# WoodOxen/tactics2d

Measured on NVIDIA H100. Metric: participant_steps_per_sec, higher is better.
Workload: dtype f32

## Files before the change

### tactics2d_b200/csrc/t2d_kernels.cu

```cuda
#include <cuda_runtime.h>
#include <stdint.h>
#include <stdio.h>
#include <string.h>

#include <algorithm>
#include <atomic>
#include <cmath>
#include <memory>
#include <mutex>
#include <string>
#include <vector>

#include "../../include/t2d_b200.h"
#include "t2d_math.cuh"

namespace t2d {

constexpr int MAX_WARPS_PER_CTA = 8;
constexpr int CTA_THREADS = MAX_WARPS_PER_CTA * 32;
constexpr int PPL = 4;
constexpr int POSE_PER_WARP = 32 * PPL;
constexpr int MAP_SMEM_LIMIT = 120 * 1024;

struct MapHeader {
// ... 13 lines not shown
  uint32_t smem_bytes;
  float bxmin, bxmax, bymin, bymax;
  int32_t has_bounds;
  uint32_t pad[3];
};
constexpr float CLEAR_QUANT = 0.125f;
static_assert(sizeof(MapHeader) == 128, "MapHeader must be 128 bytes");

struct WorldArgs {
  float *x, *y, *h, *v, *vx, *vy;
  const uint8_t* type_id;
  int32_t* step_count;
  const Params* table;
  int n_types, N, M;
};

struct MapArgs {
  const unsigned char* map_blob;
  const uint32_t* tile_off;
  const uint16_t* tile_id;
};

__device__ __forceinline__ const unsigned char* tile_blob(const MapArgs& m, long long n) {
  return m.map_blob ? m.map_blob + (m.tile_id ? m.tile_off[m.tile_id[n]] : 0u) : nullptr;
}

struct GoalArgs {
  const float* target;
  float* iou;
  float* last_pose;
  int32_t* noact_count;
  float threshold;
  int noact_max;
};

struct StepArgs {
  float *x, *y, *h, *v, *vx, *vy;
  const uint8_t* type_id;
  int32_t* step_count;
  const float* action;
  const float* ego_action;
  uint8_t* flags;
  int16_t* hit_index;
  int16_t* hit_segment;
  uint8_t* scn_status;
  uint8_t* done;
  const unsigned char* map_blob;
  const uint32_t* tile_off;
  const uint16_t* tile_id;
  MapHeader mh;
  const Params* table;
  int map_bytes, map_in_smem;
  int n_types;
  int N, M, G;
  int g_shift, mp_shift, unused1, n_tiles, wpc, table_bytes;
  int off_poseA, off_poseB, off_hit, off_queue, off_sorted, unused0, off_qcount, off_bar;
  int n_steps;
  float dt, dt_rem;
  double dt_d, dt_rem_d, interval_d;
  int max_step, cfg_flags;
  int do_physics, has_bounds, vec_ok, needs_vel_in;
  int prefetch;
  float bxmin, bxmax, bymin, bymax;
  float rb_max;
  GoalArgs goal;
  float *wheel_f, *wheel_r;
};

__device__ __forceinline__ uint32_t smem_u32(const void* p) { return (uint32_t)__cvta_generic_to_shared(p); }

__device__ __forceinline__ void mbar_init(uint64_t* bar, uint32_t count) {
  asm volatile("mbarrier.init.shared::cta.b64 [%0], %1;" ::"r"(smem_u32(bar)), "r"(count));
}
__device__ __forceinline__ void fence_mbar_init() { asm volatile("fence.mbarrier_init.release.cluster;" ::: "memory"); }
__device__ __forceinline__ void mbar_expect_tx(uint64_t* bar, uint32_t bytes) {
  asm volatile("mbarrier.arrive.expect_tx.shared::cta.b64 _, [%0], %1;" ::"r"(smem_u32(bar)), "r"(bytes) : "memory");
}
__device__ __forceinline__ void bulk_g2s(void* dst, const void* src, uint32_t bytes, uint64_t* bar) {
  asm volatile("cp.async.bulk.shared::cluster.global.mbarrier::complete_tx::bytes [%0], [%1], %2, [%3];" ::"r"(
                   smem_u32(dst)),
               "l"(src), "r"(bytes), "r"(smem_u32(bar))
               : "memory");
}
__device__ __forceinline__ void mbar_wait(uint64_t* bar, uint32_t parity) {
  uint32_t ok = 0;
  while (!ok) {
    asm volatile(
        "{\n\t.reg .pred p;\n\t"
        "mbarrier.try_wait.parity.shared::cta.b64 p, [%1], %2;\n\t"
        "selp.u32 %0, 1, 0, p;\n\t}"
        : "=r"(ok)
        : "r"(smem_u32(bar)), "r"(parity)
        : "memory");
  }
}

template <int BYTES> struct VecOf;
template <> struct VecOf<1> { using T = uint8_t; };
template <> struct VecOf<2> { using T = uint16_t; };
template <> struct VecOf<4> { using T = uint32_t; };
template <> struct VecOf<8> { using T = uint2; };
template <> struct VecOf<16> { using T = uint4; };

template <typename T, int N>
__device__ __forceinline__ void ld_vec(const T* p, T (&o)[N]) {
  using V = typename VecOf<sizeof(T) * N>::T;
  const V v = *reinterpret_cast<const V*>(p);
  memcpy(o, &v, sizeof(V));
}
template <typename T, int N>
__device__ __forceinline__ void st_vec(T* p, const T (&o)[N]) {
  using V = typename VecOf<sizeof(T) * N>::T;
  V v;
  memcpy(&v, o, sizeof(V));
  *reinterpret_cast<V*>(p) = v;
}

struct Pose {
  float x, y, h, c, s, l, w;
};

__device__ __noinline__ bool pair_exact(const Pose a, const Pose b) {
  const bool ca = a.w < 0.0f, cb = b.w < 0.0f;
  if (!ca && !cb) return obb_obb_f64(a.x, a.y, a.h, a.l, a.w, b.x, b.y, b.h, b.l, b.w);
  if (!ca && cb) return obb_circle_f64(a.x, a.y, a.h, a.l, a.w, b.x, b.y, b.l);
  if (ca && !cb) return obb_circle_f64(b.x, b.y, b.h, b.l, b.w, a.x, a.y, a.l);
  return circle_circle_f64(a.x, a.y, a.l, b.x, b.y, b.l);
}

__device__ __forceinline__ bool pair_hit(const Pose& a, const Pose& b) {
  const bool ca = a.w < 0.0f, cb = b.w < 0.0f;
  int r;
  if (!ca && !cb) r = obb_obb_f32(a.x, a.y, a.c, a.s, a.l, a.w, b.x, b.y, b.c, b.s, b.l, b.w);
  else if (!ca && cb) r = obb_circle_f32(a.x, a.y, a.c, a.s, a.l, a.w, b.x, b.y, b.l);
  else if (ca && !cb) r = obb_circle_f32(b.x, b.y, b.c, b.s, b.l, b.w, a.x, a.y, a.l);
  else r = circle_circle_f32(a.x, a.y, a.l, b.x, b.y, b.l);
  if (r < 0) return pair_exact(a, b);
  return r != 0;
}

__device__ __noinline__ bool seg_exact(const Pose a, const float4 sg) {
  if (a.w < 0.0f) return circle_segment_f64(a.x, a.y, a.l, sg.x, sg.y, sg.z, sg.w);
  return obb_segment_f64(a.x, a.y, a.h, a.l, a.w, sg.x, sg.y, sg.z, sg.w);
}

__device__ __forceinline__ bool seg_hit(const Pose& a, const float4 sg) {
  int r = a.w < 0.0f ? circle_segment_f32(a.x, a.y, a.l, sg.x, sg.y, sg.z, sg.w)
                     : obb_segment_f32(a.x, a.y, a.c, a.s, a.l, a.w, sg.x, sg.y, sg.z, sg.w);
  if (r < 0) return seg_exact(a, sg);
  return r != 0;
}

__device__ __noinline__ bool oob_exact(const Pose a, float xmin, float xmax, float ymin, float ymax) {
  return out_of_bound_f64(a.x, a.y, a.h, a.l, a.w, a.w < 0.0f, xmin, xmax, ymin, ymax);
}

__device__ __noinline__ void other_model_step(OneIO& io, const Params& p, int n_steps, double dt, double dt_rem, double interval) {
  if (p.model() == MODEL_DYNAMICS) {
    dynamics_step(io, p, n_steps, dt);
  } else if (p.model() == MODEL_POINTMASS_NEWTON) {
    pointmass_newton_step(io, p, interval);
  } else if (p.model() == MODEL_POINTMASS_EULER) {
    pointmass_euler_step(io, p, n_steps, dt, dt_rem);
  } else {
    sincos_fast(io.h, &io.sh, &io.ch);
  }
// ... 206 lines not shown
    return t;
  };
  __syncwarp();
  for (int k = lane; k < base; k += 32) {
    const int ti = (int)queue[k];
    const TileRef t = tile_of(ti);
    const Pose a = load_pose(poseA, poseB, ti);
    const int best = t.mh->n_seg > 0 ? static_walk(ti, a, poseA[pslot(ti)].z, *t.mh, map_view(t.sec, *t.mh), queue, qcount) : 0x7fffffff;
    segmin[pslot(ti)] = best;
  }
  __syncwarp();
  const int n_x = min(*qcount, QCAP - QX0);
  for (int k = lane; k < n_x; k += 32) {
    const unsigned e = queue[QX0 + k];
    const int ti = (int)(e >> 16), sidx = (int)(e & 0xffffu);
    int* sm = &segmin[pslot(ti)];
    if (*sm != -2 && sidx < *sm) {
      const TileRef t = tile_of(ti);
      if (seg_exact(load_pose(poseA, poseB, ti), reinterpret_cast<const float4*>(t.sec + t.mh->off_seg)[sidx])) atomicMin(sm, sidx);
    }
  }
  __syncwarp();
  for (int k = lane; k < base; k += 32) {
    const int ti = (int)queue[k];
    int* sm = &segmin[pslot(ti)];
    const TileRef t = tile_of(ti);
    if (*sm == -2) {
      const MapView mv = map_view(t.sec, *t.mh);
      *sm = static_walk_exact(load_pose(poseA, poseB, ti), poseA[pslot(ti)].z, *t.mh, mv.seg, mv.cell_start, mv.items);
    }
    if (t.mh->n_poly > 0) {
      const float4 pa = poseA[pslot(ti)];
      *sm = static_objects(*sm, pa.x, pa.y, *t.mh, t.blob);
    }
  }
  __syncwarp();
}

__device__ __noinline__ bool oob_slow(const float4* poseA, const float4* poseB, int idx, float xmin, float xmax, float ymin, float ymax) {
  const Pose a = load_pose(poseA, poseB, idx);
  int r = out_of_bound_f32(a.x, a.y, a.c, a.s, a.l, a.w, a.w < 0.0f, xmin, xmax, ymin, ymax);
  if (r < 0) r = out_of_bound_f64(a.x, a.y, a.h, a.l, a.w, a.w < 0.0f, xmin, xmax, ymin, ymax) ? 1 : 0;
  return r != 0;
}

template <class Args>
__device__ __noinline__ unsigned ego_goal_events(const Args& A, long long n, float ex, float ey, float eh, float el, float ew) {
  const GoalArgs& G = A.goal;
  unsigned r = 0;
  float* last = G.last_pose + 4 * n;
  if (G.noact_max > 0) {
    int cnt = G.noact_count[n];
    if (last[3] != 0.0f) {
      const double iou = rect_iou_f64(ex, ey, eh, el, ew, last[0], last[1], last[2], el, ew);
      cnt = iou > 0.999 ? cnt + 1 : 0;
    }
    G.noact_count[n] = cnt;
    if (cnt > G.noact_max) r |= 2u;
  }
  last[0] = ex; last[1] = ey; last[2] = eh; last[3] = 1.0f;
  const float* tg = G.target + 5 * n;
  const double iou = rect_iou_f64(ex, ey, eh, el, ew, tg[0], tg[1], tg[2], tg[3], tg[4]);
  G.iou[n] = (float)iou;
  if (iou >= (double)G.threshold) r |= 1u;
  return r;
}

constexpr int FIX_M = 64, FIX_G = 16, FIX_G_SHIFT = 4, FIX_MP_SHIFT = 6;

template <bool FIXED>
__device__ __forceinline__ void prefetch_tile_l2(const StepArgs& A, long long i) {
  asm volatile("prefetch.global.L2 [%0];" ::"l"(A.x + i));
  asm volatile("prefetch.global.L2 [%0];" ::"l"(A.y + i));
  asm volatile("prefetch.global.L2 [%0];" ::"l"(A.h + i));
  asm volatile("prefetch.global.L2 [%0];" ::"l"(A.v + i));
  if (FIXED || A.action) asm volatile("prefetch.global.L2 [%0];" ::"l"(A.action + 2 * i));
  asm volatile("prefetch.global.L2 [%0];" ::"l"(A.type_id + i));
  if (!FIXED && A.needs_vel_in) {
    asm volatile("prefetch.global.L2 [%0];" ::"l"(A.vx + i));
    asm volatile("prefetch.global.L2 [%0];" ::"l"(A.vy + i));
  }
}

#ifdef T2D_TICK_TIMELINE
constexpr int TL_POINTS = 9, TL_MAX_WARPS = 4096;
__device__ unsigned long long t2d_timeline[TL_MAX_WARPS][TL_POINTS][2];
#define T2D_TL(k, on, slot, dep)                                                                                    \
  do {                                                                                                              \
    if ((on) && (slot) < TL_MAX_WARPS) {                                                                            \
      unsigned long long g_, c_;                                                                                    \
      asm volatile("mov.u64 %0, %%globaltimer;\n\tmov.u64 %1, %%clock64;" : "=l"(g_), "=l"(c_) : "f"(dep) : "memory"); \
      t2d_timeline[slot][k][0] = g_;                                                                                \
      t2d_timeline[slot][k][1] = c_;                                                                                \
    }                                                                                                               \
  } while (0)
#else
#define T2D_TL(k, on, slot, dep)
#endif

template <bool KIN_ONLY, bool MAP_TABLE, bool FIXED>
__global__ void __launch_bounds__(CTA_THREADS, 2) t2d_step_kernel(const __grid_constant__ StepArgs A) {
  extern __shared__ __align__(128) unsigned char smem[];
  T2D_TL(0, (threadIdx.x & 31) == 0, (int)(blockIdx.x * A.wpc + (threadIdx.x >> 5)), 0.0f);
  const int map_smem_bytes = (!MAP_TABLE && A.map_in_smem) ? A.map_bytes : 0;
  const int table_bytes = A.table_bytes;
  const int wpc = A.wpc;
  unsigned char* s_map = smem;
  Params* s_table = reinterpret_cast<Params*>(smem + map_smem_bytes);
  float4* s_poseA = reinterpret_cast<float4*>(smem + A.off_poseA);
  float4* s_poseB = reinterpret_cast<float4*>(smem + A.off_poseB);
  int* s_hit = reinterpret_cast<int*>(smem + A.off_hit);
  unsigned* s_queue = reinterpret_cast<unsigned*>(smem + A.off_queue);
  float4* s_sorted = reinterpret_cast<float4*>(smem + A.off_sorted);
  int* s_qcount = reinterpret_cast<int*>(smem + A.off_qcount);
  uint64_t* s_bar = reinterpret_cast<uint64_t*>(smem + A.off_bar);

  const int tid = threadIdx.x, lane = tid & 31, warp = tid >> 5;
  asm volatile("griddepcontrol.launch_dependents;" ::: "memory");

  if (tid == 0) {
    mbar_init(s_bar, 1);
    fence_mbar_init();
  }
  __syncthreads();
  if (tid == 0) {
    mbar_expect_tx(s_bar, (uint32_t)(table_bytes + map_smem_bytes));
    bulk_g2s(s_table, A.table, (uint32_t)table_bytes, s_bar);
    if (map_smem_bytes > 0) bulk_g2s(s_map, A.map_blob, (uint32_t)map_smem_bytes, s_bar);
  }
  bool staged = false;
#define K1_SHAPE(field, fixed_value) (FIXED ? (fixed_value) : A.field)
  {
    const long long n_ = ((long long)blockIdx.x * wpc + warp) * (32 >> K1_SHAPE(g_shift, FIX_G_SHIFT)) + (lane >> K1_SHAPE(g_shift, FIX_G_SHIFT));
    const int m_ = (lane & (K1_SHAPE(G, FIX_G) - 1)) * PPL;
    if (A.prefetch && n_ < A.N && m_ < K1_SHAPE(M, FIX_M)) prefetch_tile_l2<FIXED>(A, n_ * K1_SHAPE(M, FIX_M) + m_);
  }
  asm volatile("griddepcontrol.wait;" ::: "memory");
  T2D_TL(1, lane == 0, (int)blockIdx.x * wpc + warp, 0.0f);
  const int G = K1_SHAPE(G, FIX_G), M = K1_SHAPE(M, FIX_M);
  const int spw = 32 >> K1_SHAPE(g_shift, FIX_G_SHIFT);
  const int sub = lane >> K1_SHAPE(g_shift, FIX_G_SHIFT);
  const int gl = lane & (G - 1);
  const int m0 = gl * PPL;
  const int MP = G * PPL;
  float4* poseA = s_poseA + warp * POSE_PER_WARP;
  float4* poseB = s_poseB + warp * POSE_PER_WARP;
  int* hitmin = s_hit + warp * POSE_PER_WARP;
  unsigned* queue = s_queue + warp * QCAP;
  int* qcount = s_qcount + warp;
  const int tb = sub * MP, t0 = tb + m0;
  const int mp_shift = K1_SHAPE(mp_shift, FIX_MP_SHIFT);
  float4* sorted = s_sorted + warp * POSE_PER_WARP + tb;
  const int Mh = M >> 1;

  const int n_tiles = A.n_tiles;
  for (int tile = (int)blockIdx.x * wpc + warp; tile < n_tiles; tile += (int)gridDim.x * wpc) {
    const long long n = (long long)tile * spw + sub;
    const bool scn_ok = n < A.N;
    int nvalid = scn_ok ? (FIXED ? PPL : min(PPL, M - m0)) : 0;
    if (nvalid < 0) nvalid = 0;
    const long long idx0 = n * M + m0;
#ifdef T2D_TICK_TIMELINE
    const bool tl_on = lane == 0 && tile == (int)blockIdx.x * wpc + warp;
    const int tl_slot = tile;
#endif

    float sx[PPL], sy[PPL], shd[PPL], sv[PPL], svx[PPL], svy[PPL], a0[PPL], a1[PPL];
    int tidv[PPL];
#pragma unroll
    for (int i = 0; i < PPL; ++i) {
      sx[i] = sy[i] = shd[i] = sv[i] = svx[i] = svy[i] = a0[i] = a1[i] = 0.0f;
      tidv[i] = T2D_TYPE_INACTIVE;
    }
    if (nvalid == PPL && K1_SHAPE(vec_ok, 1)) {
      ld_vec<float, PPL>(A.x + idx0, sx);
      ld_vec<float, PPL>(A.y + idx0, sy);
      ld_vec<float, PPL>(A.h + idx0, shd);
      ld_vec<float, PPL>(A.v + idx0, sv);
      uint8_t tb8[PPL];
      ld_vec<uint8_t, PPL>(A.type_id + idx0, tb8);
#pragma unroll
      for (int i = 0; i < PPL; ++i) tidv[i] = tb8[i];
      if (K1_SHAPE(do_physics, 1)) {
        float2 act[PPL];
        float lo[4], hi[4];
        ld_vec<float, 4>(A.action + 2 * idx0, lo);
        ld_vec<float, 4>(A.action + 2 * idx0 + 4, hi);
        act[0] = make_float2(lo[0], lo[1]); act[1] = make_float2(lo[2], lo[3]);
        act[2] = make_float2(hi[0], hi[1]); act[3] = make_float2(hi[2], hi[3]);
#pragma unroll
        for (int i = 0; i < PPL; ++i) { a0[i] = act[i].x; a1[i] = act[i].y; }
        if (K1_SHAPE(needs_vel_in, 0)) {
          ld_vec<float, PPL>(A.vx + idx0, svx);
          ld_vec<float, PPL>(A.vy + idx0, svy);
        }
      }
    } else {
#pragma unroll
      for (int i = 0; i < PPL; ++i) {
        if (i < nvalid) {
          sx[i] = A.x[idx0 + i]; sy[i] = A.y[idx0 + i]; shd[i] = A.h[idx0 + i]; sv[i] = A.v[idx0 + i];
          tidv[i] = A.type_id[idx0 + i];
          if (K1_SHAPE(do_physics, 1)) {
            a0[i] = A.action[2 * (idx0 + i)]; a1[i] = A.action[2 * (idx0 + i) + 1];
            if (K1_SHAPE(needs_vel_in, 0)) { svx[i] = A.vx[idx0 + i]; svy[i] = A.vy[idx0 + i]; }
          }
        }
      }
    }
    {
      const long long n_next = n + (long long)gridDim.x * wpc * spw;
      if (A.prefetch && n_next < A.N && m0 < M) prefetch_tile_l2<FIXED>(A, n_next * M + m0);
    }
    if (K1_SHAPE(ego_action, nullptr) != nullptr && K1_SHAPE(do_physics, 1) && gl == 0 && scn_ok) {
      const float2 ea = reinterpret_cast<const float2*>(K1_SHAPE(ego_action, nullptr))[n];
      a0[0] = ea.x; a1[0] = ea.y;
    }
    if (!staged) {
      mbar_wait(s_bar, 0);
      staged = true;
    }
    float ch[PPL], sh[PPL];
    bool active[PPL], kin[PPL];
    const Params* pp[PPL];
    int model[PPL];
    bool lane_all_kin = true, lane_any_kin = false;
#pragma unroll
    for (int i = 0; i < PPL; ++i) {
      active[i] = tidv[i] < A.n_types;
      pp[i] = &s_table[active[i] ? tidv[i] : 0];
      model[i] = pp[i]->model_shape & 0xff;
      kin[i] = active[i] && (model[i] == MODEL_KINEMATICS);
      lane_all_kin = lane_all_kin && kin[i];
      lane_any_kin = lane_any_kin || kin[i];
      ch[i] = 1.0f; sh[i] = 0.0f;
    }
    T2D_TL(2, tl_on, tl_slot, sx[PPL - 1] + sy[PPL - 1] + shd[PPL - 1] + sv[PPL - 1] + a0[PPL - 1] + a1[PPL - 1] + (float)model[PPL - 1]);
    if (A.cfg_flags & T2D_CFG_STEER_FIRST) {
#pragma unroll
      for (int i = 0; i < PPL; ++i)
        if (model[i] <= MODEL_DYNAMICS || model[i] == MODEL_DRIFT) { float t = a0[i]; a0[i] = a1[i]; a1[i] = t; }
    }

    if (K1_SHAPE(do_physics, 1)) {
      if (__any_sync(0xffffffffu, lane_any_kin)) {
        const Params* const null_row = &s_table[A.n_types];
        const Params* pk[PPL];
        KinIO<PPL> io;
#pragma unroll
        for (int i = 0; i < PPL; ++i) {
          pk[i] = kin[i] ? pp[i] : null_row;
          io.x[i] = kin[i] ? sx[i] : 0.0f; io.y[i] = kin[i] ? sy[i] : 0.0f;
          io.h[i] = kin[i] ? shd[i] : 0.0f; io.v[i] = kin[i] ? sv[i] : 0.0f;
          io.acc[i] = kin[i] ? a0[i] : 0.0f; io.steer[i] = kin[i] ? a1[i] : 0.0f;
        }
        kinematics_step<PPL>(io, pk, A.n_steps, A.dt, A.dt_rem);
#pragma unroll
// ... 186 lines not shown
        if (((solid_bits >> i) & 1u) && near_decide(near_q[i], near_alt[i], rb[i])) near_bits |= 1u << i;
      if (__any_sync(0xffffffffu, near_bits != 0)) {
        static_phase<MAP_TABLE>(near_bits, t0, lane, tile * spw, mp_shift, A, s_map, poseA, poseB, hitmin, queue, qcount);
#pragma unroll
        for (int i = 0; i < PPL; ++i) {
          const int h = hitmin[i * 32 + lane];
          hseg[i] = (h == 0x7fffffff) ? -1 : h;
        }
      }
    }
    T2D_TL(7, tl_on, tl_slot, (float)(hseg[0] + hseg[PPL - 1]));

    float bxmin = A.bxmin, bxmax = A.bxmax, bymin = A.bymin, bymax = A.bymax;
    bool has_bounds = A.has_bounds != 0;
    if constexpr (MAP_TABLE) {
      has_bounds = lane_mh->has_bounds != 0;
      bxmin = lane_mh->bxmin; bxmax = lane_mh->bxmax; bymin = lane_mh->bymin; bymax = lane_mh->bymax;
    }
    uint8_t fl[PPL];
    unsigned oob_check = 0;
#pragma unroll
    for (int i = 0; i < PPL; ++i) {
      uint8_t f = 0;
      if (hit[i] >= 0) f |= T2D_F_DYNAMIC;
      if (hseg[i] >= 0) f |= T2D_F_STATIC;
      const float r = rb[i] * 1.0001f + 1e-3f;
      const bool clear_in = (px[i] - bxmin > r) && (bxmax - px[i] > r) && (py[i] - bymin > r) && (bymax - py[i] > r);
      if (has_bounds && ((solid_bits >> i) & 1u) && !clear_in) oob_check |= 1u << i;
      fl[i] = f;
    }
    if (oob_check) {
#pragma unroll
      for (int i = 0; i < PPL; ++i)
        if (((oob_check >> i) & 1u) && oob_slow(poseA, poseB, t0 + i, bxmin, bxmax, bymin, bymax)) fl[i] |= T2D_F_OUTBOUND;
    }
    if (nvalid == PPL && K1_SHAPE(vec_ok, 1)) {
      int16_t h16[PPL], s16[PPL];
#pragma unroll
      for (int i = 0; i < PPL; ++i) { h16[i] = (int16_t)hit[i]; s16[i] = (int16_t)hseg[i]; }
      if (A.flags) st_vec<uint8_t, PPL>(A.flags + idx0, fl);
      if (A.hit_index) st_vec<int16_t, PPL>(A.hit_index + idx0, h16);
      if (A.hit_segment) st_vec<int16_t, PPL>(A.hit_segment + idx0, s16);
    } else {
#pragma unroll
      for (int i = 0; i < PPL; ++i) {
        if (i < nvalid) {
          if (A.flags) A.flags[idx0 + i] = fl[i];
          if (A.hit_index) A.hit_index[idx0 + i] = (int16_t)hit[i];
          if (A.hit_segment) A.hit_segment[idx0 + i] = (int16_t)hseg[i];
        }
      }
    }

    if (K1_SHAPE(do_physics, 1)) {
      unsigned agg;
      if (A.cfg_flags & T2D_CFG_ANY_PARTICIPANT) {
        agg = 0;
#pragma unroll
        for (int i = 0; i < PPL; ++i) agg |= fl[i];
        for (int o = G >> 1; o > 0; o >>= 1) agg |= __shfl_xor_sync(0xffffffffu, agg, o);
      } else {
        agg = __shfl_sync(0xffffffffu, (unsigned)fl[0], sub * G);
      }
      if (gl == 0 && scn_ok) {
        const int cnt = cnt_in + 1;
        A.step_count[n] = cnt;
        uint8_t st = T2D_STATUS_NORMAL;
        unsigned goal = 0;
        if (K1_SHAPE(goal.target, nullptr) != nullptr) {
          const float4 ea = poseA[pslot(t0)], eb = poseB[pslot(t0)];
          if (ea.x == ea.x && eb.w >= 0.0f) goal = ego_goal_events(A, n, ea.x, ea.y, ea.w, eb.z, eb.w);
        }
        if (goal & 1u) st = T2D_STATUS_COMPLETED;
        if (agg & T2D_F_DYNAMIC) st = T2D_STATUS_FAILED;
        if (agg & T2D_F_STATIC) st = T2D_STATUS_FAILED;
        if (agg & T2D_F_OUTBOUND) st = T2D_STATUS_OUT_BOUND;
        if (goal & 2u) st = T2D_STATUS_NO_ACTION;
        if (A.max_step > 0 && cnt > A.max_step) st = T2D_STATUS_TIME_EXCEEDED;
        if (A.scn_status) A.scn_status[n] = st;
        if (A.done) A.done[n] = st != T2D_STATUS_NORMAL;
      }
    }
    T2D_TL(8, tl_on, tl_slot, 0.0f);
    __syncwarp();
  }
  if (!staged) mbar_wait(s_bar, 0);
#undef K1_SHAPE
}

struct ResetArgs : WorldArgs {
  const uint8_t* mask;
  const int32_t* pool_index;
  const float *px, *py, *ph, *pv, *pvx, *pvy;
  GoalArgs goal;
  float *wheel_f, *wheel_r;
  const float *pool_wf, *pool_wr;
  float* last_accel;
  int n_pool;
  uint8_t* agent_type_id;
  uint8_t* agent_retired;
  GoalArgs agent;
  int agent_q;
};

__global__ void t2d_reset_kernel(const __grid_constant__ ResetArgs A) {
  const long long total = (long long)A.N * A.M;
  for (long long i = (long long)blockIdx.x * blockDim.x + threadIdx.x; i < total; i += (long long)gridDim.x * blockDim.x) {
    const int n = (int)(i / A.M), m = (int)(i - (long long)n * A.M);
    if (!A.mask[n]) continue;
    int r = A.pool_index ? A.pool_index[n] : n;
    r = min(max(r, 0), A.n_pool - 1);
    const long long s = (long long)r * A.M + m;
    A.x[i] = A.px[s]; A.y[i] = A.py[s]; A.h[i] = A.ph[s]; A.v[i] = A.pv[s];
    A.vx[i] = A.pvx ? A.pvx[s] : A.pv[s] * cosf(A.ph[s]);
    A.vy[i] = A.pvy ? A.pvy[s] : A.pv[s] * sinf(A.ph[s]);
    if (A.agent_type_id != nullptr) {
      const uint8_t rt = A.agent_retired[i];
      if (rt != 0xff) { A.agent_type_id[i] = rt; A.agent_retired[i] = 0xff; }
      for (int q = m; q < A.agent_q; q += A.M) {
        A.agent.last_pose[4 * ((long long)n * A.agent_q + q) + 3] = 0.0f;
        A.agent.noact_count[(long long)n * A.agent_q + q] = 0;
      }
    }
    if (A.wheel_f != nullptr) {
      float wf = 0.0f, wr = 0.0f;
      if (A.pool_wf != nullptr) {
        wf = A.pool_wf[s]; wr = A.pool_wr[s];
      } else {
        const int tid = A.type_id[i];
        if (tid < A.n_types && A.table[tid].model() == MODEL_DRIFT) wf = wr = A.pv[s] / A.table[tid].wheel_radius;
      }
      A.wheel_f[i] = wf; A.wheel_r[i] = wr;
    }
    if (A.last_accel != nullptr) A.last_accel[i] = 0.0f;
    if (m == 0) {
      A.step_count[n] = 0;
      if (A.goal.last_pose) A.goal.last_pose[4 * (long long)n + 3] = 0.0f;
      if (A.goal.noact_count) A.goal.noact_count[n] = 0;
    }
  }
}

struct EnvArgs : WorldArgs {
  const uint8_t* flags;
  const uint8_t* status;
  const float* iou;
  const float* target;
  float* max_iou;
  float* min_dist;
  float* reward;
  uint8_t *terminated, *truncated, *done;
  uint8_t* traffic_status;
  int max_step, reset_trackers;
};

__device__ __noinline__ float reward_chain(int st, int ts, int step_count, int max_step, float iou, float* max_iou,
                                           const float* target, float* min_dist, float x, float y) {
  float r;
  if (ts == 3 || ts == 4) r = -5.0f;
  else if (st == T2D_STATUS_TIME_EXCEEDED || st == T2D_STATUS_NO_ACTION) r = -1.0f;
  else if (st == T2D_STATUS_OUT_BOUND) r = -5.0f;
  else if (st == T2D_STATUS_COMPLETED) r = 5.0f;
  else {
    r = max_step > 0 ? -tanhf((float)step_count / (float)max_step) * 0.001f : 0.0f;
    if (max_iou != nullptr) {
      const float best = *max_iou;
      r += (best == -INFINITY) ? iou : iou - best;
// ... 1404 lines not shown

static int launch_replay(t2d_ctx* c, void* stream, int first, int count, int offset, const uint8_t* mask, const int32_t* pool_index) {
  const DeviceLog& g = *c->log;
  if (g.type_id != c->type_id) return fail(T2D_E_STATE, "state rebound after t2d_set_log: call t2d_set_log again");
  const size_t p0 = (size_t)first * c->M;
  ReplayArgs R{};
  R.x = c->x + p0; R.y = c->y + p0; R.h = c->h + p0; R.v = c->v + p0; R.vx = c->vx + p0; R.vy = c->vy + p0;
  R.type_id = g.type_id + p0;
  R.step_count = c->step_count + first;
  R.log_row = g.row + first;
  R.mask = mask ? mask + first : nullptr;
  R.pool_index = pool_index ? pool_index + first : nullptr;
  R.log_row_out = mask ? g.row + first : nullptr;
  R.tracks = g.tracks.get(); R.track_type = g.track_type.get(); R.rec = g.rec.get();
  R.t0 = g.t0.get(); R.slot_off = g.slot_off.get(); R.entries = g.entries.get(); R.slot_track1 = g.slot_track1.get();
  R.track_out = g.track_out ? g.track_out + p0 : nullptr;
  R.N = count; R.M = c->M; R.n_rows = g.n_rows; R.offset = offset; R.interval_ms = c->cfg.interval_ms;
  t2d_replay_kernel<<<capped_grid((long long)count * c->M, 256, c->sm_count, 8), 256, 0, (cudaStream_t)stream>>>(R);
  return launched();
}

static bool aligned16(const void* p) { return (reinterpret_cast<uintptr_t>(p) & 15) == 0; }

static int pick_wpc(long long tiles, int sm_count) {
  const int resident_warps = 14;
  if (tiles > (long long)sm_count * resident_warps) return MAX_WARPS_PER_CTA;
  int best = 2;
  double best_cost = 1e30;
  for (int w = 2; w <= MAX_WARPS_PER_CTA; ++w) {
    const long long ctas = (tiles + w - 1) / w;
    const long long per_sm = (ctas + sm_count - 1) / sm_count;
    const double cost = (double)(per_sm * w) + 0.42 * (double)per_sm;
    if (cost < best_cost - 1e-9 || (cost < best_cost + 1e-9 && w > best)) { best_cost = cost; best = w; }
  }
  return best;
}

static int launch_step(t2d_ctx* c, const float* action, const float* ego, uint8_t* flags, int16_t* hit_index, int16_t* hit_segment,
                       uint8_t* scn_status, uint8_t* done, void* stream, int do_physics, int first = 0, int count = -1) {
  if (!c) return fail(T2D_E_INVALID, "ctx is NULL");
  if (int r = require(c, NEED_STATE | NEED_TABLE)) return r;
  if (do_physics && !action) return fail(T2D_E_INVALID, "action is NULL");
  if (do_physics)
    if (int r = require(c, NEED_TICK)) return r;
  CUDA_TRY(cudaSetDevice(c->device));
  if (count < 0) count = c->N - first;
  if (first < 0 || count <= 0 || first + count > c->N) return fail(T2D_E_INVALID, "scenario range out of bounds");
  const DeviceMap& map = c->map;
  const size_t p0 = (size_t)first * c->M;
  StepArgs A{};
  A.x = c->x + p0; A.y = c->y + p0; A.h = c->h + p0; A.v = c->v + p0; A.vx = c->vx + p0; A.vy = c->vy + p0;
  A.type_id = c->type_id + p0; A.step_count = c->step_count + first;
  A.wheel_f = c->wheel_f ? c->wheel_f + p0 : nullptr; A.wheel_r = c->wheel_r ? c->wheel_r + p0 : nullptr;
  A.action = action; A.ego_action = ego ? ego + 2 * (size_t)first : nullptr; A.flags = flags; A.hit_index = hit_index; A.hit_segment = hit_segment;
  A.scn_status = scn_status; A.done = done;
  const bool map_table = map.n_tiles > 1;
  const MapArgs mp = map_args(map, first);
  A.map_blob = mp.map_blob; A.tile_off = mp.tile_off; A.tile_id = mp.tile_id; A.map_bytes = map.smem_bytes; A.mh = map.mh;
  A.map_in_smem = (!map_table && map.blob && map.mh.n_seg > 0 && map.smem_bytes <= MAP_SMEM_LIMIT) ? 1 : 0;
  A.table = c->d_table.get(); A.n_types = c->n_types;
  A.N = count; A.M = c->M; A.G = c->G;
  set_time_step(A, c->cfg.interval_ms, c->cfg.delta_t_ms);
  A.max_step = c->cfg.max_step; A.cfg_flags = c->cfg.flags;
  A.do_physics = do_physics; A.has_bounds = map.has_bounds ? 1 : 0;
  A.bxmin = map.mh.bxmin; A.bxmax = map.mh.bxmax; A.bymin = map.mh.bymin; A.bymax = map.mh.bymax;
  A.prefetch = c->prefetch_override >= 0 ? c->prefetch_override : (g_exchanges_alive.load() == 0 ? 1 : 0);
  A.needs_vel_in = (c->has_pointmass || c->has_drift || (do_physics && c->log)) ? 1 : 0;
  bool vec = (c->M % PPL == 0) && aligned16(A.x) && aligned16(A.y) && aligned16(A.h) && aligned16(A.v) && aligned16(A.vx) &&
             aligned16(A.vy) && (reinterpret_cast<uintptr_t>(A.type_id) % 4 == 0) && (!action || aligned16(action)) &&
             (!flags || reinterpret_cast<uintptr_t>(flags) % 4 == 0) && (!hit_index || reinterpret_cast<uintptr_t>(hit_index) % 8 == 0) &&
             (!hit_segment || reinterpret_cast<uintptr_t>(hit_segment) % 8 == 0);
  A.vec_ok = vec ? 1 : 0;

  A.rb_max = c->rb_max;
  A.goal = c->goal;
  if (A.goal.target) {
    A.goal.target += 5 * (size_t)first; A.goal.iou += first; A.goal.last_pose += 4 * (size_t)first; A.goal.noact_count += first;
  }
  const int table_bytes = (((c->n_types + 1) * (int)sizeof(Params) + 15) / 16) * 16;
  const int spw = 32 / c->G;
  const long long tiles = ((long long)count + spw - 1) / spw;
  int wpc = pick_wpc(tiles, c->sm_count);
  if (c->wpc_override > 0) wpc = c->wpc_override;
  {
    int off = (A.map_in_smem ? A.map_bytes : 0) + table_bytes;
    A.off_poseA = off; off += wpc * POSE_PER_WARP * (int)sizeof(float4);
    A.off_poseB = off; off += wpc * POSE_PER_WARP * (int)sizeof(float4);
    A.off_hit = off; off += wpc * POSE_PER_WARP * (int)sizeof(int);
    A.off_queue = off; off += wpc * QCAP * 4;
    A.off_sorted = off; off += wpc * POSE_PER_WARP * (int)sizeof(float4);
    A.off_qcount = off; off += ((wpc + 3) & ~3) * 4;
    A.off_bar = off; off += 16;
    A.wpc = wpc;
    A.table_bytes = table_bytes;
    A.n_tiles = (int)tiles;
    A.g_shift = 0;
    while ((1 << A.g_shift) < c->G) ++A.g_shift;
    const int MP = c->G * PPL;
    A.mp_shift = 0;
    while ((1 << A.mp_shift) < MP) ++A.mp_shift;
  }
  const int smem = A.off_bar + 16;
  if (smem > c->max_smem_optin) return fail(T2D_E_UNSUPPORTED, "shared memory budget exceeded");
  using kernel_t = void (*)(StepArgs);
  kernel_t kern;
  const bool fixed = c->kin_only && !c->tick_generic && c->M == FIX_M && c->G == FIX_G && do_physics && A.vec_ok &&
                     !A.needs_vel_in && A.ego_action == nullptr && A.goal.target == nullptr;
  if (fixed) kern = map_table ? (kernel_t)t2d_step_kernel<true, true, true> : (kernel_t)t2d_step_kernel<true, false, true>;
  else if (c->kin_only) kern = map_table ? (kernel_t)t2d_step_kernel<true, true, false> : (kernel_t)t2d_step_kernel<true, false, false>;
  else kern = map_table ? (kernel_t)t2d_step_kernel<false, true, false> : (kernel_t)t2d_step_kernel<false, false, false>;
  const int variant = (fixed ? 4 : c->kin_only ? 2 : 0) + (map_table ? 1 : 0);
  {
    std::lock_guard<std::mutex> lock(g_smem_mutex);
    int& configured = g_smem_configured[c->device % 64][variant];
    if (smem > configured) {
      CUDA_TRY(cudaFuncSetAttribute(kern, cudaFuncAttributeMaxDynamicSharedMemorySize, smem));
      configured = smem;
    }
  }
  if (do_physics && c->log)
    if (int r = launch_replay(c, stream, first, count, 1, nullptr, nullptr)) return r;
  if (do_physics && c->has_drift) {
    t2d_drift_kernel<<<capped_grid((long long)count * c->M, 128, c->sm_count, 16), 128, 0, (cudaStream_t)stream>>>(A);
    if (int r = launched()) return r;
  }
  const long long ctas_needed = (tiles + wpc - 1) / wpc;
  if (c->occ_smem[wpc] != smem || c->occ_variant[wpc] != variant) {
    int per_sm = 1;
    CUDA_TRY(cudaOccupancyMaxActiveBlocksPerMultiprocessor(&per_sm, kern, wpc * 32, smem));
    c->occ_val[wpc] = per_sm < 1 ? 1 : per_sm;
    c->occ_smem[wpc] = smem;
    c->occ_variant[wpc] = variant;
  }
  int per_sm_ctas = c->occ_val[wpc];
  if (c->grid_limit > 0) per_sm_ctas = std::min(per_sm_ctas, c->grid_limit);
  const long long resident = (long long)c->sm_count * per_sm_ctas;
  const int grid = (int)std::max(1LL, std::min(ctas_needed, resident));
  cudaLaunchConfig_t cfg{};
  cfg.gridDim = dim3((unsigned)grid);
  cfg.blockDim = dim3((unsigned)(wpc * 32));
  cfg.dynamicSmemBytes = (size_t)smem;
  cfg.stream = (cudaStream_t)stream;
  cudaLaunchAttribute attr[1];
  attr[0].id = cudaLaunchAttributeProgrammaticStreamSerialization;
  attr[0].val.programmaticStreamSerializationAllowed = c->use_pdl ? 1 : 0;
  cfg.attrs = attr;
  cfg.numAttrs = 1;
  CUDA_TRY(cudaLaunchKernelEx(&cfg, kern, A));
  if (int r = launched()) return r;
  g_tick_instances[variant].fetch_add(1);
  if (!map_table && map.blob && map.mh.n_seg > 0 && !A.map_in_smem) g_tick_instances[6].fetch_add(1);
  return T2D_OK;
}

static int launch_control(t2d_ctx* c, float* action, const float* ego, void* stream) {
  if (int r = require(c, NEED_STATE | NEED_TABLE)) return r;
  if (!c->d_ctab) return fail(T2D_E_STATE, "controllers not set: call t2d_set_controllers first");
  if (!action) return fail(T2D_E_INVALID, "action is NULL");
  if (reinterpret_cast<uintptr_t>(action) % 8 != 0) return fail(T2D_E_INVALID, "action must be 8-byte aligned");
  CUDA_TRY(cudaSetDevice(c->device));
  CtrlArgs A{world_args(c)};
  A.ctab = c->d_ctab.get(); A.n_ctrl = c->n_ctrl; A.ctrl_id = c->ctrl_id; A.lead = c->ctrl_lead; A.path_id = c->ctrl_path;
  A.path_v = c->d_path_v.get(); A.path_off = c->d_path_off.get(); A.n_paths = c->n_paths;
  A.last_accel = c->ctrl_last_accel; A.action = action; A.ego_action = ego;
  A.steer_first = (c->cfg.flags & T2D_CFG_STEER_FIRST) ? 1 : 0;
  const int warps_per_cta = 4;
  t2d_control_kernel<<<capped_grid(c->N, warps_per_cta, c->sm_count, 16), warps_per_cta * 32, 0, (cudaStream_t)stream>>>(A);
  return launched();
}

struct HostPart {
  void* dst;
  size_t off, bytes;
};

static int read_back(const Mirror& m, size_t bytes, cudaStream_t s, std::initializer_list<HostPart> parts) {
  CUDA_TRY(cudaMemcpyAsync(m.host.get(), m.dev.get(), bytes, cudaMemcpyDeviceToHost, s));
  CUDA_TRY(cudaStreamSynchronize(s));
  for (const HostPart& p : parts)
    if (p.dst) memcpy(p.dst, m.host.get() + p.off, p.bytes);
  return T2D_OK;
}

static int make_mirror(Mirror& out, size_t dev_bytes, size_t host_bytes) {
  Mirror m;
  if (int r = dev_alloc(m.dev, dev_bytes)) return r;
  if (int r = host_alloc(m.host, host_bytes)) return r;
  out = std::move(m);
  return T2D_OK;
}
// ... 608 lines not shown
```

Before: 15.36 billion.

## Stage fixed-shape tile inputs into shared memory via per-warp TMA bulk copies

```diff
diff --git a/tactics2d_b200/csrc/t2d_kernels.cu b/tactics2d_b200/csrc/t2d_kernels.cu
--- a/tactics2d_b200/csrc/t2d_kernels.cu
+++ b/tactics2d_b200/csrc/t2d_kernels.cu
@@ -119,6 +119,7 @@
                "l"(src), "r"(bytes), "r"(smem_u32(bar))
                : "memory");
 }
+__device__ __forceinline__ void fence_proxy_async_smem() { asm volatile("fence.proxy.async.shared::cta;" ::: "memory"); }
 __device__ __forceinline__ void mbar_wait(uint64_t* bar, uint32_t parity) {
   uint32_t ok = 0;
   while (!ok) {
@@ -491,6 +492,18 @@
   }
 }
 
+__device__ __forceinline__ void stage_tile(const StepArgs& A, int tile, float4* poseA, float4* poseB, uint64_t* bar) {
+  const long long p = (long long)tile * (2 * FIX_M);
+  const uint32_t np = (2LL * tile + 1 < A.N) ? 2 * FIX_M : FIX_M;
+  mbar_expect_tx(bar, np * (4 * sizeof(float) + 2 * sizeof(float) + 1));
+  bulk_g2s(poseB + 2 * 32, A.type_id + p, np, bar);
+  bulk_g2s(poseB, A.action + 2 * p, np * 2 * sizeof(float), bar);
+  bulk_g2s(poseA + 2 * 32, A.h + p, np * sizeof(float), bar);
+  bulk_g2s(poseA + 3 * 32, A.v + p, np * sizeof(float), bar);
+  bulk_g2s(poseA, A.x + p, np * sizeof(float), bar);
+  bulk_g2s(poseA + 32, A.y + p, np * sizeof(float), bar);
+}
+
 #ifdef T2D_TICK_TIMELINE
 constexpr int TL_POINTS = 9, TL_MAX_WARPS = 4096;
 __device__ unsigned long long t2d_timeline[TL_MAX_WARPS][TL_POINTS][2];
@@ -529,6 +542,8 @@
 
   if (tid == 0) {
     mbar_init(s_bar, 1);
+    if constexpr (FIXED)
+      for (int w = 0; w < wpc; ++w) mbar_init(s_bar + 1 + w, 1);
     fence_mbar_init();
   }
   __syncthreads();
@@ -545,6 +560,14 @@
     if (A.prefetch && n_ < A.N && m_ < K1_SHAPE(M, FIX_M)) prefetch_tile_l2<FIXED>(A, n_ * K1_SHAPE(M, FIX_M) + m_);
   }
   asm volatile("griddepcontrol.wait;" ::: "memory");
+  if constexpr (FIXED) {
+    if (tid == 0)
+      for (int w = 0; w < wpc; ++w) {
+        const int t = (int)blockIdx.x * wpc + w;
+        if (t < A.n_tiles) stage_tile(A, t, s_poseA + w * POSE_PER_WARP, s_poseB + w * POSE_PER_WARP, s_bar + 1 + w);
+      }
+  }
+  uint32_t tile_parity = 0;
   T2D_TL(1, lane == 0, (int)blockIdx.x * wpc + warp, 0.0f);
   const int G = K1_SHAPE(G, FIX_G), M = K1_SHAPE(M, FIX_M);
   const int spw = 32 >> K1_SHAPE(g_shift, FIX_G_SHIFT);
@@ -581,7 +604,24 @@
       sx[i] = sy[i] = shd[i] = sv[i] = svx[i] = svy[i] = a0[i] = a1[i] = 0.0f;
       tidv[i] = T2D_TYPE_INACTIVE;
     }
-    if (nvalid == PPL && K1_SHAPE(vec_ok, 1)) {
+    if constexpr (FIXED) {
+      mbar_wait(s_bar + 1 + warp, tile_parity);
+      tile_parity ^= 1u;
+      if (nvalid == PPL) {
+        const float4 fx = poseA[lane], fy = poseA[32 + lane], fh = poseA[2 * 32 + lane], fv = poseA[3 * 32 + lane];
+        const float4 lo = poseB[2 * lane], hi = poseB[2 * lane + 1];
+        const uint32_t t4 = reinterpret_cast<const uint32_t*>(poseB + 2 * 32)[lane];
+        sx[0] = fx.x; sx[1] = fx.y; sx[2] = fx.z; sx[3] = fx.w;
+        sy[0] = fy.x; sy[1] = fy.y; sy[2] = fy.z; sy[3] = fy.w;
+        shd[0] = fh.x; shd[1] = fh.y; shd[2] = fh.z; shd[3] = fh.w;
+        sv[0] = fv.x; sv[1] = fv.y; sv[2] = fv.z; sv[3] = fv.w;
+        a0[0] = lo.x; a1[0] = lo.y; a0[1] = lo.z; a1[1] = lo.w;
+        a0[2] = hi.x; a1[2] = hi.y; a0[3] = hi.z; a1[3] = hi.w;
+#pragma unroll
+        for (int i = 0; i < PPL; ++i) tidv[i] = (t4 >> (8 * i)) & 0xffu;
+      }
+      __syncwarp();
+    } else if (nvalid == PPL && K1_SHAPE(vec_ok, 1)) {
       ld_vec<float, PPL>(A.x + idx0, sx);
       ld_vec<float, PPL>(A.y + idx0, sy);
       ld_vec<float, PPL>(A.h + idx0, shd);
@@ -934,7 +974,12 @@
       }
     }
     T2D_TL(8, tl_on, tl_slot, 0.0f);
+    if constexpr (FIXED) fence_proxy_async_smem();
     __syncwarp();
+    if constexpr (FIXED) {
+      const int next = tile + (int)gridDim.x * wpc;
+      if (lane == 0 && next < n_tiles) stage_tile(A, next, poseA, poseB, s_bar + 1 + warp);
+    }
   }
   if (!staged) mbar_wait(s_bar, 0);
 #undef K1_SHAPE
@@ -2505,6 +2550,8 @@
   const long long tiles = ((long long)count + spw - 1) / spw;
   int wpc = pick_wpc(tiles, c->sm_count);
   if (c->wpc_override > 0) wpc = c->wpc_override;
+  const bool fixed = c->kin_only && !c->tick_generic && c->M == FIX_M && c->G == FIX_G && do_physics && A.vec_ok &&
+                     aligned16(A.type_id) && !A.needs_vel_in && A.ego_action == nullptr && A.goal.target == nullptr;
   {
     int off = (A.map_in_smem ? A.map_bytes : 0) + table_bytes;
     A.off_poseA = off; off += wpc * POSE_PER_WARP * (int)sizeof(float4);
@@ -2513,7 +2560,7 @@
     A.off_queue = off; off += wpc * QCAP * 4;
     A.off_sorted = off; off += wpc * POSE_PER_WARP * (int)sizeof(float4);
     A.off_qcount = off; off += ((wpc + 3) & ~3) * 4;
-    A.off_bar = off; off += 16;
+    A.off_bar = off; off += 16 + (fixed ? wpc * 8 : 0);
     A.wpc = wpc;
     A.table_bytes = table_bytes;
     A.n_tiles = (int)tiles;
@@ -2523,12 +2570,10 @@
     A.mp_shift = 0;
     while ((1 << A.mp_shift) < MP) ++A.mp_shift;
   }
-  const int smem = A.off_bar + 16;
+  const int smem = A.off_bar + 16 + (fixed ? wpc * 8 : 0);
   if (smem > c->max_smem_optin) return fail(T2D_E_UNSUPPORTED, "shared memory budget exceeded");
   using kernel_t = void (*)(StepArgs);
   kernel_t kern;
-  const bool fixed = c->kin_only && !c->tick_generic && c->M == FIX_M && c->G == FIX_G && do_physics && A.vec_ok &&
-                     !A.needs_vel_in && A.ego_action == nullptr && A.goal.target == nullptr;
   if (fixed) kern = map_table ? (kernel_t)t2d_step_kernel<true, true, true> : (kernel_t)t2d_step_kernel<true, false, true>;
   else if (c->kin_only) kern = map_table ? (kernel_t)t2d_step_kernel<true, true, false> : (kernel_t)t2d_step_kernel<true, false, false>;
   else kern = map_table ? (kernel_t)t2d_step_kernel<false, true, false> : (kernel_t)t2d_step_kernel<false, false, false>;
```

New measurement: 15.39 billion, median of 6. Within noise of the previous version (+0.2%).
